# snphbaum/scikit-gpuppy

Measured on NVIDIA B200. Metric: fit_s_per_iter, lower is better.
Workload: dtype f64

## Files before the change

scikit-gpuppy_b200/csrc/factor.cuh:

```cuda
#pragma once
#include "dgemm_dmma.cuh"
#include "oz_gemm.cuh"
#include "leaf_blocked.cuh"

namespace gpk {


struct FactorCtx {
  double* A;
  double* X;
  long ld;
  double* dL;
  int* info;
  cudaStream_t st;
  cudaStream_t side = nullptr;
  cudaEvent_t* ev = nullptr;
  int* ev_next = nullptr;
  oz::Workspace* oz = nullptr;
  oz::Workspace* ovl_ws = nullptr;
  cudaStream_t* ovl_st = nullptr;
  int ovl_depths = 0;
};

inline int leaf_launch(const FactorCtx& c, int r0) {
// ... 80 lines not shown
  GPK_TRY((gemm_store_auto<LAY_KC, LAY_KC>(
      gemm_args(A21, ld, X11, ld, X21, ld, h2, h1, h1, 1.0, 0.0, K_UPTO_BJ, 0), c.st)));
  cudaStream_t tst = c.st;
  cudaEvent_t joined = nullptr;
  if (c.side) {
    cudaEvent_t forked = c.ev[(*c.ev_next)++];
    joined = c.ev[(*c.ev_next)++];
    GPK_CUDA_OK(cudaEventRecord(forked, c.st));
    GPK_CUDA_OK(cudaStreamWaitEvent(c.side, forked, 0));
    tst = c.side;
  }
  GPK_TRY((gemm_store_auto<LAY_KC, LAY_MC>(
      gemm_args(X21, ld, X11, ld, A21, ld, h2, h1, h1, 1.0, 0.0, K_FROM_BJ, 0), tst)));
  if (c.side) GPK_CUDA_OK(cudaEventRecord(joined, c.side));
  GPK_TRY((gemm_store_auto<LAY_KC, LAY_KC>(
      gemm_args(X21, ld, X21, ld, A22, ld, h2, h2, h1, -1.0, 1.0, K_FULL, 1), c.st)));
  GPK_TRY(potrf_inv_node(c, r0 + h1, h2, depth + 1));
  if (c.side) GPK_CUDA_OK(cudaStreamWaitEvent(c.st, joined, 0));
  GPK_TRY((gemm_store_auto<LAY_KC, LAY_MC>(
      gemm_args(X22, ld, A21, ld, X21, ld, h2, h1, h2, -1.0, 0.0, K_UPTO_BI, 0), c.st)));
  return 0;
}

inline int lauum_launch(const double* X, double* out, long ld, int npad, cudaStream_t st, oz::Workspace* oz = nullptr) {
  if (oz && npad >= oz->min_dim)
    return oz::gemm_f64(*oz, X, ld, 1, 1, npad, X, ld, 1, 1, npad, npad, out, ld, 1.0, 0.0, K_FROM_BI, 1, st);
  return gemm_store_auto<LAY_MC, LAY_MC>(
      gemm_args(X, ld, X, ld, out, ld, npad, npad, npad, 1.0, 0.0, K_FROM_BI, 1), st);
}

__global__ void __launch_bounds__(256) trmv_lower_kernel(const double* __restrict__ X, long ld, int npad,
                                                         const double* __restrict__ t, double* __restrict__ y) {
  const int row = blockIdx.x * 8 + (threadIdx.x >> 5);
  const int lane = threadIdx.x & 31;
  if (row >= npad) return;
  const double* Xr = X + (long)row * ld;
  double s = 0.0;
  for (int k = lane; k <= row; k += 32) s = fma(Xr[k], t[k], s);
  s = warp_sum(s);
  if (lane == 0) y[row] = s;
}

constexpr int TRMVT_ROWS = 512;
__global__ void __launch_bounds__(128) trmv_lower_T_partial_kernel(const double* __restrict__ X, long ld, int npad,
                                                                   const double* __restrict__ y,
                                                                   double* __restrict__ part) {
  const int c = blockIdx.x * 128 + threadIdx.x;
  const int r_begin = blockIdx.y * TRMVT_ROWS;
  const int r_end = min(npad, r_begin + TRMVT_ROWS);
// ... 72 lines not shown
```

scikit-gpuppy_b200/csrc/gpk.cu:

```cuda
#include "../../include/gpk.h"
#include "../../include/gpk_test.h"

#include <climits>
#include <new>
#include <vector>

#include "dgemm_dmma.cuh"
#include "factor.cuh"
#include "se_kernels.cuh"
#include "exact_kernels.cuh"
#include "periodic_kernels.cuh"

namespace gpk {
thread_local char g_err[512] = {0};
thread_local long g_launch_count = 0;
thread_local bool g_prof_on = false;
static thread_local std::vector<ProfPair> g_prof;
void prof_push(cudaEvent_t a, cudaEvent_t b) { g_prof.push_back(ProfPair{a, b}); }

struct Handle {
  int n = 0, d = 0, npad = 0;
  double *X = nullptr, *W = nullptr;
  bool own_X = false, own_W = false;
  double *x = nullptr, *xT = nullptr, *t = nullptr, *y = nullptr, *alpha = nullptr, *dL = nullptr;
// ... 10 lines not shown
  double theta[3 * MAX_D + 2];
  bool factored = false, have_inverse = false;
  bool matrix_state = false;
  double logdet = 0.0, quad = 0.0, alpha2 = 0.0;
  cudaStream_t st = nullptr;
  cudaStream_t side = nullptr;
  std::vector<cudaEvent_t> events;
  int ev_next = 0;
  bool oz_want = false;
  bool oz_on = false;
  int oz_moduli_req = 0;
  size_t oz_out_cap = 0;
  oz::Workspace oz;
  oz::Workspace ozq;
  oz::Operand xs;
  bool x_sliced = false;
  cudaStream_t chain_st = nullptr;
  std::vector<cudaStream_t> ovl_st;
  std::vector<oz::Workspace> ovl_ws;
  cudaEvent_t ev_in = nullptr, ev_out = nullptr;
  bool ovl_on = false;
  double* raw_pinned = nullptr;
  bool grad_pending = false;
};

thread_local int g_overlap_T = 1;

static void release_overlap(Handle* h) {
  for (auto& w : h->ovl_ws) w.release();
  h->ovl_ws.clear();
  for (auto& s : h->ovl_st) if (s) { cudaStreamSynchronize(s); cudaStreamDestroy(s); }
  h->ovl_st.clear();
  if (h->chain_st) { cudaStreamSynchronize(h->chain_st); cudaStreamDestroy(h->chain_st); h->chain_st = nullptr; }
  if (h->ev_in) { cudaEventDestroy(h->ev_in); h->ev_in = nullptr; }
  if (h->ev_out) { cudaEventDestroy(h->ev_out); h->ev_out = nullptr; }
  h->ovl_on = false;
}

static int ensure_overlap(Handle* h) {
  if (h->ovl_on || !h->oz_on || !g_overlap_T) return 0;
  int depths = 0;
  size_t need = 0;
  for (long hh = h->npad / 2 / TILE * TILE; hh >= h->oz.min_dim; hh = hh / 2 / TILE * TILE) {
    need += (size_t)h->oz.S * (hh + TILE) * (3 * (hh + TILE) + round_up_l(hh + TILE, 256)) + 6 * hh * sizeof(double);
    ++depths;
  }
// ... 104 lines not shown
  trmv_lower_kernel<<<(npad + 7) / 8, 256, 0, h->st>>>(h->X, npad, npad, b_pad, y);
  GPK_LAUNCH_OK();
  const int nchunks = (npad + TRMVT_ROWS - 1) / TRMVT_ROWS;
  GPK_TRY(ensure(&h->part, &h->part_elems, (size_t)nchunks * npad));
  dim3 grid(npad / 128, nchunks);
  trmv_lower_T_partial_kernel<<<grid, 128, 0, h->st>>>(h->X, npad, npad, y, h->part);
  GPK_LAUNCH_OK();
  sum_chunks_kernel<<<(npad + 255) / 256, 256, 0, h->st>>>(h->part, nchunks, npad, npad, out, 1.0, 0.0);
  GPK_LAUNCH_OK();
  return 0;
}

template <int DP>
static int launch_trace(Handle* h, int d0, int trb, int tre, double* partial) {
  const int nt = h->npad / TILE;
  const size_t smem = (size_t)2 * h->d * (TILE + 2) * sizeof(double);
  GPK_CUDA_OK(cudaFuncSetAttribute(grad_trace_kernel<DP>, cudaFuncAttributeMaxDynamicSharedMemorySize, (int)smem));
  dim3 grid(nt, tre - trb);
  grad_trace_kernel<DP><<<grid, 256, smem, h->st>>>(h->W, h->npad, h->alpha, h->x, h->n, h->d, d0, h->hyp, trb, partial);
  GPK_LAUNCH_OK();
  return 0;
}

static int trace_sums(Handle* h, int trb, int tre, double* raw_host, double* async_dst = nullptr) {
  const int d = h->d;
  const int nt = h->npad / TILE;
  for (int k = 0; k <= (h->kind == KIND_PERIODIC ? 3 * d + 2 : d + 2); ++k) raw_host[k] = 0.0;
  if (tre <= trb) return 0;
  if (h->kind != KIND_PERIODIC) {
    const int r0 = trb * TILE, r1 = (tre * TILE < h->n) ? tre * TILE : h->n;
    diag_sum_kernel<<<1, 256, 0, h->st>>>(h->W, h->npad, h->alpha, r0, r1, h->scal + 4);
    GPK_LAUNCH_OK();
    GPK_CUDA_OK(cudaMemcpyAsync(async_dst ? async_dst : raw_host + d + 1, h->scal + 4, 2 * sizeof(double),
                                cudaMemcpyDeviceToHost, h->st));
  }
  if (h->kind == KIND_PERIODIC) {
    const int DPp = d <= 4 ? 4 : d <= 8 ? 8 : 16;
    const int nc = 3 * DPp + 2;
    const long nsl = (long)nt * (tre - trb);
    GPK_TRY(ensure(&h->part, &h->part_elems, (size_t)nsl * nc + nc));
    double* psums = h->part + (size_t)nsl * nc;
    dim3 pgrid(nt, tre - trb);
    if (DPp == 4) periodic_trace_kernel<4><<<pgrid, 256, 0, h->st>>>(h->W, h->npad, h->alpha, h->x, h->n, d, h->hyp, trb, h->part);
    else if (DPp == 8) periodic_trace_kernel<8><<<pgrid, 256, 0, h->st>>>(h->W, h->npad, h->alpha, h->x, h->n, d, h->hyp, trb, h->part);
    else periodic_trace_kernel<16><<<pgrid, 256, 0, h->st>>>(h->W, h->npad, h->alpha, h->x, h->n, d, h->hyp, trb, h->part);
    GPK_LAUNCH_OK();
    col_sum_kernel<<<nc, 256, 0, h->st>>>(h->part, nsl, nc, psums);
    GPK_LAUNCH_OK();
    double ph[50];
    GPK_CUDA_OK(cudaMemcpyAsync(ph, psums, nc * sizeof(double), cudaMemcpyDeviceToHost, h->st));
    GPK_CUDA_OK(cudaStreamSynchronize(h->st));
    raw_host[0] = ph[0];
    for (int k = 0; k < d; ++k) {
      raw_host[1 + k] = ph[1 + k];
      raw_host[1 + d + k] = ph[1 + DPp + k];
      raw_host[1 + 2 * d + k] = ph[1 + 2 * DPp + k];
    }
    raw_host[3 * d + 1] = ph[3 * DPp + 1];
    raw_host[3 * d + 2] = 0.0;
    return 0;
  }
  int DP = d <= 4 ? 4 : d <= 8 ? 8 : d <= 16 ? 16 : 32;
  const long nslots = (long)nt * (tre - trb);
  const int nchunks = (d + DP - 1) / DP;
  GPK_TRY(ensure(&h->part, &h->part_elems, (size_t)nslots * (DP + 1) + (size_t)nchunks * (DP + 1)));
  double* sums = h->part + (size_t)nslots * (DP + 1);
  double host[2 * 33];
  for (int d0 = 0, ch = 0; d0 < d; d0 += DP, ++ch) {
    switch (DP) {
      case 4: GPK_TRY(launch_trace<4>(h, d0, trb, tre, h->part)); break;
      case 8: GPK_TRY(launch_trace<8>(h, d0, trb, tre, h->part)); break;
      case 16: GPK_TRY(launch_trace<16>(h, d0, trb, tre, h->part)); break;
      default: GPK_TRY(launch_trace<32>(h, d0, trb, tre, h->part)); break;
    }
    col_sum_kernel<<<DP + 1, 256, 0, h->st>>>(h->part, nslots, DP + 1, sums + ch * (DP + 1));
    GPK_LAUNCH_OK();
    double* dst = async_dst ? async_dst + 4 + ch * (DP + 1) : host + ch * 33;
    GPK_CUDA_OK(cudaMemcpyAsync(dst, sums + ch * (DP + 1), (DP + 1) * sizeof(double), cudaMemcpyDeviceToHost, h->st));
  }
  if (async_dst) return 0;
  GPK_CUDA_OK(cudaStreamSynchronize(h->st));
  for (int d0 = 0, ch = 0; d0 < d; d0 += DP, ++ch) {
    if (d0 == 0) raw_host[0] = host[0];
    for (int k = 0; k < DP && d0 + k < d; ++k) raw_host[1 + d0 + k] = host[ch * 33 + 1 + k];
  }
  return 0;
}

static void trace_unpack(const Handle* h, const double* pinned, double* raw_host) {
  const int d = h->d;
  const int DP = d <= 4 ? 4 : d <= 8 ? 8 : d <= 16 ? 16 : 32;
  raw_host[d + 1] = pinned[0];
  raw_host[d + 2] = pinned[1];
  for (int d0 = 0, ch = 0; d0 < d; d0 += DP, ++ch) {
    const double* src = pinned + 4 + ch * (DP + 1);
    if (d0 == 0) raw_host[0] = src[0];
    for (int k = 0; k < DP && d0 + k < d; ++k) raw_host[1 + d0 + k] = src[1 + k];
  }
}

static int ensure_route(Handle* h);

static int do_lauum(Handle* h) {
  if (h->have_inverse) return 0;
  GPK_TRY(ensure_route(h));
  h->x_sliced = false;
  GPK_TRY(lauum_launch(h->X, h->W, h->npad, h->npad, h->st, h->oz_on ? &h->oz : nullptr));
  h->have_inverse = true;
  return 0;
}

static bool same_theta(const Handle* h, const double* theta) {
  if (!h->factored || h->matrix_state) return false;
  return memcmp(h->theta, theta, sizeof(double) * theta_len(h->kind, h->d)) == 0;
}

static long batch_rows_for(const Handle* h, long want) {
  long cap = (long)(4.0e9 / (8.0 * h->npad));
  cap = cap / TILE * TILE;
  if (cap > 16384) cap = 16384;
  if (cap < TILE) cap = TILE;
  if (h->batch_rows > 0 && h->batch_rows < cap) cap = round_up_l(h->batch_rows, TILE);
  long r = round_up_l(want, TILE);
  return r < cap ? r : cap;
}

static int ensure_query_ws(Handle* h, long rows) {
  const long nbi = h->npad / TILE;
  GPK_TRY(ensure(&h->G, &h->G_elems, (size_t)rows * h->npad));
  size_t need = (size_t)nbi * rows + (size_t)nbi * (rows / 2);
  if (h->colsq_elems < need) {
// ... 160 lines not shown
  }
  Handle* h = new (std::nothrow) Handle();
  if (!h) return -3;
  const int rc = create_fill(h, n, d, Xbuf, Wbuf);
  if (rc != 0) {
    cudaGetLastError();
    gpk_destroy(reinterpret_cast<gpk_handle>(h));
    return rc;
  }
  *out = reinterpret_cast<gpk_handle>(h);
  return 0;
}

int gpk_destroy(gpk_handle h) {
  H_OR_FAIL(h);
  cudaStreamSynchronize(hh->st);
  if (hh->own_X) cudaFree(hh->X);
  if (hh->own_W) cudaFree(hh->W);
  cudaFree(hh->x); cudaFree(hh->xT); cudaFree(hh->t); cudaFree(hh->y); cudaFree(hh->alpha); cudaFree(hh->dL);
  cudaFree(hh->scal); cudaFree(hh->info);
  for (auto& e : hh->events) if (e) cudaEventDestroy(e);
  if (hh->side) { cudaStreamSynchronize(hh->side); cudaStreamDestroy(hh->side); }
  if (hh->part) cudaFree(hh->part);
  if (hh->G) cudaFree(hh->G);
  if (hh->colsq) cudaFree(hh->colsq);
  if (hh->dots) cudaFree(hh->dots);
  hh->oz.release();
  hh->ozq.release();
  release_overlap(hh);
  if (hh->raw_pinned) cudaFreeHost(hh->raw_pinned);
  delete hh;
  return 0;
}

int gpk_set_stream(gpk_handle h, void* stream) {
  H_OR_FAIL(h);
  hh->st = reinterpret_cast<cudaStream_t>(stream);
  return 0;
}

int gpk_set_kernel(gpk_handle h, int kind) {
  H_OR_FAIL(h);
  if (kind != KIND_SE && kind != KIND_PERIODIC) { snprintf(g_err, sizeof(g_err), "unknown kernel kind %d", kind); return -2; }
  if (kind == KIND_PERIODIC && hh->d > PER_MAX_D) {
    snprintf(g_err, sizeof(g_err), "the periodic covariance supports d <= %d", PER_MAX_D);
    return -2;
// ... 100 lines not shown
    cudaDeviceSynchronize();
    return rc_rec;
  }
  if (ovl) {
    GPK_CUDA_OK(cudaEventRecord(hh->ev_out, hh->chain_st));
    GPK_CUDA_OK(cudaStreamWaitEvent(hh->st, hh->ev_out, 0));
  }
  GPK_TRY(solve_one(hh, hh->t, hh->y, hh->alpha));
  nll_scalars_kernel<<<1, 256, 0, hh->st>>>(hh->dL, hh->y, hh->alpha, n, hh->scal);
  GPK_LAUNCH_OK();
  int info = 0;
  double sc[3];
  GPK_CUDA_OK(cudaMemcpyAsync(&info, hh->info, sizeof(int), cudaMemcpyDeviceToHost, hh->st));
  GPK_CUDA_OK(cudaMemcpyAsync(sc, hh->scal, 3 * sizeof(double), cudaMemcpyDeviceToHost, hh->st));
  GPK_CUDA_OK(cudaStreamSynchronize(hh->st));
  if (info != INT_MAX) {
    snprintf(g_err, sizeof(g_err), "leading minor %d of K is not positive definite", info);
    return info > 0 ? info : 1;
  }
  hh->logdet = sc[0]; hh->quad = sc[1]; hh->alpha2 = sc[2];
  return 0;
}

int gpk_factorize(gpk_handle h, const double* theta, int want_inverse) {
  H_OR_FAIL(h);
  if (!same_theta(hh, theta)) {
    hh->factored = false;
    hh->have_inverse = false;
    hh->x_sliced = false;
    hh->grad_pending = false;
    GPK_TRY(set_hyper(hh->hyp, theta, hh->d, hh->kind));
    GPK_TRY(ensure_route(hh));
    const int n = hh->n, npad = hh->npad;
    GPK_TRY(launch_se_tiles(hh->x, n, hh->x, n, hh->d, hh->hyp, hh->W, npad, npad, npad,
                            hh->kind == KIND_PERIODIC ? 2 : 1, 1, 1, hh->st));
    const int rc = factorize_W(hh);
    if (rc != 0) return rc;
    memcpy(hh->theta, theta, sizeof(double) * theta_len(hh->kind, hh->d));
    hh->factored = true;
    hh->matrix_state = false;
  }
  if (want_inverse) GPK_TRY(do_lauum(hh));
  return 0;
}

__global__ void __launch_bounds__(256) load_matrix_kernel(const double* __restrict__ K, long ldk, int n,
                                                          double* __restrict__ W, long ld, int npad) {
  const int c = blockIdx.x * 256 + threadIdx.x;
  const int r = blockIdx.y;
  if (c >= npad || (c >> 7) > (r >> 7)) return;
  W[(long)r * ld + c] = (r < n && c < n) ? K[(long)r * ldk + c] : (r == c ? 1.0 : 0.0);
}

int gpk_factorize_matrix(gpk_handle h, const double* K_dev, int64_t ldk, int want_inverse) {
  H_OR_FAIL(h);
  if (!K_dev || ldk < hh->n) { snprintf(g_err, sizeof(g_err), "gpk_factorize_matrix: bad matrix argument"); return -2; }
  hh->factored = false;
  hh->have_inverse = false;
  hh->x_sliced = false;
  GPK_TRY(ensure_route(hh));
  dim3 grid((hh->npad + 255) / 256, hh->npad);
  load_matrix_kernel<<<grid, 256, 0, hh->st>>>(K_dev, ldk, hh->n, hh->W, hh->npad, hh->npad);
  GPK_LAUNCH_OK();
  const int rc = factorize_W(hh);
  if (rc != 0) return rc;
  hh->factored = true;
// ... 15 lines not shown
  if (!hh->factored) { snprintf(g_err, sizeof(g_err), "not factored"); return -2; }
  *out = hh->logdet;
  return 0;
}

int gpk_grad_trace_partial(gpk_handle h, int64_t trb, int64_t tre, double* out) {
  H_OR_FAIL(h);
  if (!hh->factored || !hh->have_inverse || hh->matrix_state) { snprintf(g_err, sizeof(g_err), "inverse not available"); return -2; }
  if (hh->kind != KIND_SE) { snprintf(g_err, sizeof(g_err), "sharded trace: Gaussian covariance only"); return -2; }
  const int nt = hh->npad / TILE;
  if (trb < 0) trb = 0;
  if (tre > nt) tre = nt;
  return trace_sums(hh, (int)trb, (int)tre, out);
}

int gpk_nll_grad(gpk_handle h, const double* theta, double* nll, double* grad, int want_grad) {
  H_OR_FAIL(h);
  const bool prefetch = want_grad == 2 && hh->kind == KIND_SE;
  const bool cached = same_theta(hh, theta);
  if (!cached && hh->grad_pending) {
    GPK_CUDA_OK(cudaStreamSynchronize(hh->st));
    hh->grad_pending = false;
  }
  int rc = gpk_factorize(h, theta, want_grad == 1);
  if (rc != 0) return rc;
  const double two_pi = 6.283185307179586476925286766559;
  if (nll) *nll = 0.5 * hh->n * log(two_pi) + 0.5 * hh->logdet + 0.5 * hh->quad;
  if (prefetch && !hh->grad_pending) {
    if (!hh->raw_pinned) GPK_CUDA_OK(cudaMallocHost((void**)&hh->raw_pinned, (3 * MAX_D + 8) * sizeof(double)));
    GPK_TRY(do_lauum(hh));
    double unused[3 * MAX_D + 3];
    GPK_TRY(trace_sums(hh, 0, hh->npad / TILE, unused, hh->raw_pinned));
    hh->grad_pending = true;
    return 0;
  }
  if (want_grad == 1 && grad) {
    double raw[3 * MAX_D + 3];
    if (hh->grad_pending) {
      GPK_CUDA_OK(cudaStreamSynchronize(hh->st));
      trace_unpack(hh, hh->raw_pinned, raw);
      hh->grad_pending = false;
    } else {
      GPK_TRY(trace_sums(hh, 0, hh->npad / TILE, raw));
    }
    const int d = hh->d;
    grad[0] = 0.5 * raw[0];
    if (hh->kind == KIND_PERIODIC) {
      grad[1] = 0.5 * hh->hyp.vt * raw[3 * d + 1];
      for (int k = 0; k < d; ++k) {
        grad[2 + k] = -0.25 * hh->hyp.w[k] * raw[1 + k];
        grad[2 + d + k] = 0.5 * hh->hyp.pf[k] * hh->hyp.w2[k] * raw[1 + d + k];
        grad[2 + 2 * d + k] = -0.25 * hh->hyp.w2[k] * raw[1 + 2 * d + k];
      }
      return 0;
    }
    grad[1] = 0.5 * hh->hyp.vt * (raw[hh->d + 1] - raw[hh->d + 2]);
    for (int k = 0; k < hh->d; ++k) grad[2 + k] = -0.25 * hh->hyp.w[k] * raw[1 + k];
  }
  return 0;
}

int gpk_solve(gpk_handle h, const double* b, int64_t nrhs, double* out) {
  H_OR_FAIL(h);
  if (!hh->factored) { snprintf(g_err, sizeof(g_err), "not factored"); return -2; }
  const int npad = hh->npad, n = hh->n;
  GPK_TRY(ensure_query_ws(hh, TILE));
// ... 457 lines not shown
```

scikit-gpuppy_b200/csrc/oz_crt_planes.cuh:

```cuda

struct PlaneArgs {
  uint8_t* res; long res_ld; long res_plane;
  int M, N, K;
  int row_tile0;
  int krange, lower_only;
  int widen, band_cols;
  int nmod;
  unsigned int* phase;
  int* spill;
  int m[CRT_MAX_MODULI]; uint32_t magic[CRT_MAX_MODULI]; uint32_t u[CRT_MAX_MODULI];
};

constexpr int RECON_GROUPS = (CRT_MAX_MODULI + 3) / 4;

struct ReconArgs {
  const uint8_t* res; long res_ld; long res_plane;
  double* C; long ldc;
  const double* scA; const double* scB;
  double alpha, beta;
  int M, N, K;
  int row0;
  int krange, lower_only;
  int nmod;
  double p_scaled;
  double* colsq; double* pairdot; long ldo;
  uint32_t wp[2 * RECON_GROUPS][6];
};

constexpr int SPILL_SLOTS = 256;
constexpr int Q_BN = 256;
constexpr int Q_STAGES = 7;
constexpr int Q_STAGE_BYTES = 2 * TILE_BYTES;
constexpr int Q_SMEM_BYTES = Q_STAGES * Q_STAGE_BYTES + 1024 + 256;

__host__ __device__ __forceinline__ void planes_krange(int krange, int K, int bi2, int bx2, int& kb0, int& kb1) {
  kb0 = 0;
  kb1 = K / BK;
  switch (krange) {
    case K_UPTO_BJ: kb1 = (kb1 < 2 * bx2 + 2) ? kb1 : 2 * bx2 + 2; break;
    case K_FROM_BJ: kb0 = (kb1 < 2 * bx2) ? kb1 : 2 * bx2; break;
    case K_UPTO_BI: kb1 = (kb1 < 2 * bi2 + 2) ? kb1 : 2 * bi2 + 2; break;
    case K_FROM_BI: kb0 = (kb1 < 2 * bi2) ? kb1 : 2 * bi2; break;
    default: break;
  }
}

__global__ void __launch_bounds__(THREADS, 1)
oz_crt_planes_kernel(const __grid_constant__ CUtensorMap tmA, const __grid_constant__ CUtensorMap tmB,
                     const __grid_constant__ PlaneArgs p) {
  extern __shared__ uint8_t oz_smem_raw[];
// ... 205 lines not shown
        o[1] = make_uint4(pk[4], pk[5], pk[6], pk[7]);
      }
    }
  }
#undef SEG_MOD
#undef SEG_BEG
#undef SEG_END
  tc_fence_before();
  cluster_sync_all();
  if (warp == 2) tmem_dealloc_pair(tmem_base, TMEM_COLS);
}

__device__ __forceinline__ uint32_t dp2a_lo(uint32_t a, uint32_t b, uint32_t c) {
  uint32_t d;
  asm("dp2a.lo.u32.u32 %0, %1, %2, %3;" : "=r"(d) : "r"(a), "r"(b), "r"(c));
  return d;
}
__device__ __forceinline__ uint32_t dp2a_hi(uint32_t a, uint32_t b, uint32_t c) {
  uint32_t d;
  asm("dp2a.hi.u32.u32 %0, %1, %2, %3;" : "=r"(d) : "r"(a), "r"(b), "r"(c));
  return d;
}

template <int EPI, int NG>
__global__ void __launch_bounds__(256, 4) oz_crt_reconstruct_kernel(const __grid_constant__ ReconArgs p) {
  const int lane = threadIdx.x & 31, warp = threadIdx.x >> 5;
  const int bjc = blockIdx.x;
  const long lrow = (long)blockIdx.y * 8 + warp;
  const long grow = (long)p.row0 + lrow;
  const long gcol = (long)bjc * 128 + lane * 4;
  const int bi = (int)(grow >> 7), bi2 = (int)(grow >> 8), bx2 = bjc >> 1;
  if (EPI == OZ_EPI_STORE && p.lower_only && bjc > bi) return;
  int kb0, kb1;
  planes_krange(p.krange, p.K, bi2, bx2, kb0, kb1);
  const bool computed = (kb1 > kb0) && !(p.lower_only && 2 * bx2 > 2 * bi2 + 1);

  uint32_t acc[4][6];
#pragma unroll
  for (int x = 0; x < 4; ++x)
#pragma unroll
    for (int j = 0; j < 6; ++j) acc[x][j] = 0u;
  if (computed) {
    const uint8_t* src = p.res + lrow * p.res_ld + gcol;
    uint32_t q[NG * 4];
#pragma unroll
    for (int i = 0; i < NG * 4; ++i) {
      q[i] = (i < 4 * (NG - 1) || i < p.nmod) ? __ldcs(reinterpret_cast<const uint32_t*>(src)) : 0u;
      src += p.res_plane;
    }
#pragma unroll
    for (int g = 0; g < NG; ++g) {
      {
        const uint32_t ab_lo = __byte_perm(q[4 * g], q[4 * g + 1], 0x5140), ab_hi = __byte_perm(q[4 * g], q[4 * g + 1], 0x7362);
        const uint32_t cd_lo = __byte_perm(q[4 * g + 2], q[4 * g + 3], 0x5140),
                       cd_hi = __byte_perm(q[4 * g + 2], q[4 * g + 3], 0x7362);
        const uint32_t t[4] = {__byte_perm(ab_lo, cd_lo, 0x5410), __byte_perm(ab_lo, cd_lo, 0x7632),
                               __byte_perm(ab_hi, cd_hi, 0x5410), __byte_perm(ab_hi, cd_hi, 0x7632)};
#pragma unroll
        for (int e = 0; e < 4; ++e)
#pragma unroll
          for (int j = 0; j < 6; ++j) {
            uint32_t v = acc[e][j];
            v = dp2a_lo(p.wp[2 * g][j], t[e], v);
            v = dp2a_hi(p.wp[2 * g + 1][j], t[e], v);
            acc[e][j] = v;
          }
      }
    }
  }
  const bool row_ok = grow < p.M;
  const bool col_ok = gcol < p.N;
  const double sa = row_ok ? p.scA[grow] * p.p_scaled : 0.0;
  double v[4];
#pragma unroll
  for (int x = 0; x < 4; ++x) {
    const unsigned long long t0 = ((unsigned long long)acc[x][1] << 16) + acc[x][0];
    const unsigned long long t1 = ((unsigned long long)acc[x][3] << 16) + acc[x][2] + (t0 >> 32);
    const unsigned long long t2 = ((unsigned long long)acc[x][5] << 16) + acc[x][4] + (t1 >> 32);
    const long long hi = (long long)((t2 << 32) | (t1 & 0xffffffffull));
    const double frac = fma((double)hi, 4294967296.0, (double)(uint32_t)t0);
    v[x] = col_ok ? sa * p.scB[gcol + x] * frac : 0.0;
  }
  if (EPI == OZ_EPI_STORE) {
    if (row_ok && col_ok) {
      double* crow = p.C + grow * p.ldc + gcol;
#pragma unroll
      for (int x = 0; x < 4; x += 2) {
        double2 o;
        o.x = p.alpha * v[x];
        o.y = p.alpha * v[x + 1];
        if (p.beta != 0.0) {
          const double2 old = *reinterpret_cast<const double2*>(crow + x);
          o.x = fma(p.beta, old.x, o.x);
          o.y = fma(p.beta, old.y, o.y);
        }
        *reinterpret_cast<double2*>(crow + x) = o;
      }
    }
  } else {
    __shared__ double vrow[8][128];
#pragma unroll
    for (int x = 0; x < 4; ++x) vrow[warp][lane * 4 + x] = v[x];
    __syncthreads();
    double sq = 0.0, pd = 0.0;
#pragma unroll
    for (int x = 0; x < 4; ++x) {
      sq = fma(v[x], v[x], sq);
      pd = fma(v[x], vrow[warp ^ 1][lane * 4 + x], pd);
    }
#pragma unroll
    for (int off = 1; off < 32; off <<= 1) {
      sq += __shfl_xor_sync(0xffffffffu, sq, off);
      pd += __shfl_xor_sync(0xffffffffu, pd, off);
    }
    if (lane == 0 && row_ok) {
      p.colsq[(long)bjc * p.ldo + grow] = sq;
      if (!(grow & 1)) p.pairdot[(long)bjc * (p.ldo / 2) + (grow >> 1)] = pd;
    }
  }
}
```

scikit-gpuppy_b200/csrc/oz_gemm.cuh:

```cuda
#pragma once
#include <cuda.h>

#include "dgemm_dmma.cuh"
#include "oz_crt_tables.h"

namespace gpk {
namespace oz {

constexpr int BM = 128, BN = 128, BK = 128;
constexpr int TILE_BYTES = BM * BK;
constexpr int EPI_WARPS = 8;
constexpr int THREADS = 64 + EPI_WARPS * 32;
constexpr int TMEM_COLS = 512;

constexpr int OZ_EPI_STORE = 0;
constexpr int OZ_EPI_ROWSQ = 1;

__device__ __forceinline__ uint32_t smem_u32(const void* p) { return (uint32_t)__cvta_generic_to_shared(p); }

__device__ __forceinline__ void mbar_init(uint64_t* bar, uint32_t count) {
  asm volatile("mbarrier.init.shared::cta.b64 [%0], %1;" ::"r"(smem_u32(bar)), "r"(count) : "memory");
}
__device__ __forceinline__ void fence_barrier_init() {
  asm volatile("fence.mbarrier_init.release.cluster;" ::: "memory");
}
__device__ __forceinline__ void mbar_expect_tx(uint64_t* bar, uint32_t bytes) {
  asm volatile("mbarrier.arrive.expect_tx.shared::cta.b64 _, [%0], %1;" ::"r"(smem_u32(bar)), "r"(bytes) : "memory");
}
__device__ __forceinline__ void mbar_arrive(uint64_t* bar) {
  asm volatile("mbarrier.arrive.shared::cta.b64 _, [%0];" ::"r"(smem_u32(bar)) : "memory");
}
__device__ __forceinline__ bool mbar_try_wait(uint64_t* bar, uint32_t parity) {
  uint32_t ok;
  asm volatile(
      "{\n\t.reg .pred p;\n\t"
      "mbarrier.try_wait.parity.shared::cta.b64 p, [%1], %2;\n\t"
      "selp.u32 %0, 1, 0, p;\n\t}\n"
      : "=r"(ok)
      : "r"(smem_u32(bar)), "r"(parity)
// ... 317 lines not shown
  if (!trans) {
    oz_absmax_rows_kernel<<<op.rows, 256, 0, st>>>(src, ld, op.K, lower, mx);
    GPK_LAUNCH_OK();
    const long chunks = (long)op.rows * (op.K >> 4);
    oz_residue_rows_kernel<<<(unsigned)((chunks + 255) / 256), 256, 0, st>>>(src, ld, op.rows, op.K, lower, op.S,
                                                                            op.bits, zero_fill_extra(op.K), mx, op.sl, op.sc);
    GPK_LAUNCH_OK();
  } else {
    GPK_CUDA_OK(cudaMemsetAsync(mx, 0, (size_t)op.rows * sizeof(unsigned long long), st));
    dim3 g1(op.rows / 32, (op.K + 1023) / 1024);
    oz_absmax_cols_kernel<<<g1, 256, 0, st>>>(src, ld, op.K, lower, mx);
    GPK_LAUNCH_OK();
    dim3 g2(op.rows / 32, (op.K + 127) / 128);
    oz_residue_cols_kernel<<<g2, 256, 0, st>>>(src, ld, op.rows, op.K, lower, op.S, op.bits, zero_fill_extra(op.K), mx, op.sl, op.sc);
    GPK_LAUNCH_OK();
  }
  return 0;
}

thread_local int g_position_lock = 2;

inline int gemm_sliced(const Operand& A, const Operand& B, double* C, long ldc, double alpha, double beta, int krange,
                       int lower_only, cudaStream_t st, int epi = OZ_EPI_STORE, double* colsq = nullptr,
                       double* pairdot = nullptr, long ldo = 0) {
  if (A.K != B.K || A.S != B.S) {
    snprintf(g_err, sizeof(g_err), "gemm_sliced: operand mismatch K %d/%d moduli %d/%d", A.K, B.K, A.S, B.S);
    return -2;
  }
  if (A.bits != B.bits || A.bits != crt_bits(A.K, A.S)) {
    snprintf(g_err, sizeof(g_err), "gemm_sliced: operand widths %d/%d do not match K=%d", A.bits, B.bits, A.K);
    return -2;
  }
  const long Nc = ((long)B.rows + Q_BN - 1) / Q_BN * Q_BN;
  const size_t per_row = (size_t)A.S * (size_t)Nc;
  const long panel = (long)(A.out_cap / per_row) / 256 * 256;
  if (!A.out || panel < 256) {
    snprintf(g_err, sizeof(g_err), "gemm_sliced: the residue-plane buffer (%zu bytes) cannot hold a 256-row panel of %ld columns",
             A.out_cap, Nc);
    return -4;
  }
  static bool configured_on[GPK_MAX_DEVICES] = {};
  bool& configured = configured_on[current_device_slot()];
  if (!configured) {
    GPK_CUDA_OK(cudaFuncSetAttribute(oz_crt_planes_kernel, cudaFuncAttributeMaxDynamicSharedMemorySize, Q_SMEM_BYTES));
    configured = true;
  }
  CUtensorMap tmA, tmB;
  GPK_TRY(make_tmap(&tmA, A.sl, A.rows, A.K, A.S, BM));
  GPK_TRY(make_tmap(&tmB, B.sl, B.rows, B.K, B.S, BM));
  const CrtSet& cs = crt_set(A.S);
  PlaneArgs g;
  memset(&g, 0, sizeof(g));
  g.res = A.out; g.res_ld = Nc;
// ... 38 lines not shown
    r.row0 = (int)row0;
    r.res_plane = g.res_plane;
    long ncol_tiles = Nc / Q_BN;
    if (lower_only && (row0 + rows_pad) / Q_BN < ncol_tiles) ncol_tiles = (row0 + rows_pad) / Q_BN;
    g.phase = phase_dev + (phase_next++ & 63);
    GPK_CUDA_OK(cudaMemsetAsync(g.phase, 0, sizeof(unsigned int), st));
    cudaLaunchConfig_t cfg;
    memset(&cfg, 0, sizeof(cfg));
    cudaLaunchAttribute attr[1];
    attr[0].id = cudaLaunchAttributeClusterDimension;
    attr[0].val.clusterDim.x = 2;
    attr[0].val.clusterDim.y = 1;
    attr[0].val.clusterDim.z = 1;
    cfg.gridDim = dim3((unsigned)(2 * ncol_tiles), (unsigned)(rows_pad / 256));
    cfg.blockDim = dim3(THREADS);
    cfg.dynamicSmemBytes = Q_SMEM_BYTES;
    cfg.stream = st;
    cfg.attrs = attr;
    cfg.numAttrs = 1;
    GPK_CUDA_OK(cudaLaunchKernelEx(&cfg, oz_crt_planes_kernel, tmA, tmB, g));
    GPK_LAUNCH_OK();
    long ncol_blocks = B.rows / 128;
    if (lower_only && (row0 + rows) / 128 < ncol_blocks) ncol_blocks = (row0 + rows) / 128;
    dim3 rg((unsigned)ncol_blocks, (unsigned)(rows / 8));
    const int ng = (A.S + 3) / 4;
    const bool store = epi == OZ_EPI_STORE;
    auto kernel = (ng <= 2) ? (store ? oz_crt_reconstruct_kernel<OZ_EPI_STORE, 2> : oz_crt_reconstruct_kernel<OZ_EPI_ROWSQ, 2>)
                : (ng == 3) ? (store ? oz_crt_reconstruct_kernel<OZ_EPI_STORE, 3> : oz_crt_reconstruct_kernel<OZ_EPI_ROWSQ, 3>)
                : (ng == 4) ? (store ? oz_crt_reconstruct_kernel<OZ_EPI_STORE, 4> : oz_crt_reconstruct_kernel<OZ_EPI_ROWSQ, 4>)
                            : (store ? oz_crt_reconstruct_kernel<OZ_EPI_STORE, 5> : oz_crt_reconstruct_kernel<OZ_EPI_ROWSQ, 5>);
    kernel<<<rg, 256, 0, st>>>(r);
    GPK_LAUNCH_OK();
  }
  if (g_prof_on) {
    GPK_CUDA_OK(cudaEventRecord(e1, st));
    prof_push(e0, e1);
  }
  return 0;
}

struct Workspace {
  int8_t* buf = nullptr; size_t cap = 0, top = 0;
  double* sc = nullptr; size_t sc_cap = 0, sc_top = 0;
  unsigned long long* mx = nullptr; size_t mx_cap = 0;
  uint8_t* out = nullptr; size_t out_cap = 0;
  int S = CRT_MIN_MODULI;
  int min_dim = 2048;
  void reset() { top = 0; sc_top = 0; }
// ... 26 lines not shown
      sc = nullptr; sc_cap = 0;
      if (cudaMalloc((void**)&sc, rows_total * sizeof(double)) != cudaSuccess) { cudaGetLastError(); return -1; }
      sc_cap = rows_total;
    }
    if (rows_max > mx_cap) {
      if (mx) cudaFree(mx);
      mx = nullptr; mx_cap = 0;
      if (cudaMalloc((void**)&mx, rows_max * sizeof(unsigned long long)) != cudaSuccess) { cudaGetLastError(); return -1; }
      mx_cap = rows_max;
    }
    return 0;
  }
  void release() {
    if (buf) cudaFree(buf);
    if (sc) cudaFree(sc);
    if (mx) cudaFree(mx);
    if (out) cudaFree(out);
    buf = nullptr; sc = nullptr; mx = nullptr; out = nullptr; cap = sc_cap = mx_cap = out_cap = 0;
  }
};

inline int gemm_f64(Workspace& ws, const double* A, long lda, int transA, int lowerA, int M, const double* B, long ldb,
                    int transB, int lowerB, int N, int K, double* C, long ldc, double alpha, double beta, int krange,
                    int lower_only, cudaStream_t st) {
  ws.reset();
  Operand a = ws.alloc(M, K);
  const bool same = (A == B && lda == ldb && transA == transB && lowerA == lowerB && M == N);
  Operand b = same ? a : ws.alloc(N, K);
  if (!a.sl || !b.sl) {
    snprintf(g_err, sizeof(g_err), "gemm_f64: residue workspace too small for %d x %d and %d x %d operands", M, K, N, K);
    return -4;
  }
  GPK_TRY(slice_operand(A, lda, transA, lowerA, a, ws.mx, st));
  if (same) b = a;
  else GPK_TRY(slice_operand(B, ldb, transB, lowerB, b, ws.mx, st));
  return gemm_sliced(a, b, C, ldc, alpha, beta, krange, lower_only, st);
}

}
}
```

Before: 0.3087.

## Fuse gradient trace reduction into INT8 CRT reconstruction epilogue of LAUUM

Adds a reconstruct kernel for the Ozaki INT8 LAUUM that, while writing K^-1 tiles, also accumulates the squared-exponential gradient trace sums per tile into a partial buffer. trace_sums then skips the separate grad_trace_kernel pass and only column-sums the fused partials. The aim is to avoid re-reading the full K^-1 matrix from memory for the gradient. In exchange the reconstruct kernel does more per-thread work with higher register and shared-memory use, and the partial buffer needs a memset on every call.

```diff
diff --git a/scikit-gpuppy_b200/csrc/factor.cuh b/scikit-gpuppy_b200/csrc/factor.cuh
--- a/scikit-gpuppy_b200/csrc/factor.cuh
+++ b/scikit-gpuppy_b200/csrc/factor.cuh
@@ -126,9 +126,14 @@
   return 0;
 }
 
-inline int lauum_launch(const double* X, double* out, long ld, int npad, cudaStream_t st, oz::Workspace* oz = nullptr) {
+inline int lauum_launch(const double* X, double* out, long ld, int npad, cudaStream_t st, oz::Workspace* oz = nullptr,
+                        const oz::TraceArgs* trace = nullptr) {
   if (oz && npad >= oz->min_dim)
-    return oz::gemm_f64(*oz, X, ld, 1, 1, npad, X, ld, 1, 1, npad, npad, out, ld, 1.0, 0.0, K_FROM_BI, 1, st);
+    return oz::gemm_f64(*oz, X, ld, 1, 1, npad, X, ld, 1, 1, npad, npad, out, ld, 1.0, 0.0, K_FROM_BI, 1, st, trace);
+  if (trace) {
+    snprintf(g_err, sizeof(g_err), "lauum_launch: the trace epilogue needs the INT8 route");
+    return -2;
+  }
   return gemm_store_auto<LAY_MC, LAY_MC>(
       gemm_args(X, ld, X, ld, out, ld, npad, npad, npad, 1.0, 0.0, K_FROM_BI, 1), st);
 }
diff --git a/scikit-gpuppy_b200/csrc/gpk.cu b/scikit-gpuppy_b200/csrc/gpk.cu
--- a/scikit-gpuppy_b200/csrc/gpk.cu
+++ b/scikit-gpuppy_b200/csrc/gpk.cu
@@ -56,6 +56,8 @@
   bool ovl_on = false;
   double* raw_pinned = nullptr;
   bool grad_pending = false;
+  double* tpart = nullptr; size_t tpart_elems = 0;
+  bool inverse_traced = false;
 };
 
 thread_local int g_overlap_T = 1;
@@ -206,11 +208,15 @@
   return 0;
 }
 
-static int trace_sums(Handle* h, int trb, int tre, double* raw_host, double* async_dst = nullptr) {
+static int trace_sums(Handle* h, int trb, int tre, double* raw_host, double* async_dst = nullptr, bool fused = false) {
   const int d = h->d;
   const int nt = h->npad / TILE;
   for (int k = 0; k <= (h->kind == KIND_PERIODIC ? 3 * d + 2 : d + 2); ++k) raw_host[k] = 0.0;
   if (tre <= trb) return 0;
+  if (fused && (!h->inverse_traced || trb != 0 || tre != nt || h->kind != KIND_SE || d > oz::TRACE_MAX_D)) {
+    snprintf(g_err, sizeof(g_err), "trace_sums: no gradient sums were formed with this K^-1");
+    return -2;
+  }
   if (h->kind != KIND_PERIODIC) {
     const int r0 = trb * TILE, r1 = (tre * TILE < h->n) ? tre * TILE : h->n;
     diag_sum_kernel<<<1, 256, 0, h->st>>>(h->W, h->npad, h->alpha, r0, r1, h->scal + 4);
@@ -251,13 +257,15 @@
   double* sums = h->part + (size_t)nslots * (DP + 1);
   double host[2 * 33];
   for (int d0 = 0, ch = 0; d0 < d; d0 += DP, ++ch) {
-    switch (DP) {
-      case 4: GPK_TRY(launch_trace<4>(h, d0, trb, tre, h->part)); break;
-      case 8: GPK_TRY(launch_trace<8>(h, d0, trb, tre, h->part)); break;
-      case 16: GPK_TRY(launch_trace<16>(h, d0, trb, tre, h->part)); break;
-      default: GPK_TRY(launch_trace<32>(h, d0, trb, tre, h->part)); break;
-    }
-    col_sum_kernel<<<DP + 1, 256, 0, h->st>>>(h->part, nslots, DP + 1, sums + ch * (DP + 1));
+    if (!fused) {
+      switch (DP) {
+        case 4: GPK_TRY(launch_trace<4>(h, d0, trb, tre, h->part)); break;
+        case 8: GPK_TRY(launch_trace<8>(h, d0, trb, tre, h->part)); break;
+        case 16: GPK_TRY(launch_trace<16>(h, d0, trb, tre, h->part)); break;
+        default: GPK_TRY(launch_trace<32>(h, d0, trb, tre, h->part)); break;
+      }
+    }
+    col_sum_kernel<<<DP + 1, 256, 0, h->st>>>(fused ? h->tpart : h->part, nslots, DP + 1, sums + ch * (DP + 1));
     GPK_LAUNCH_OK();
     double* dst = async_dst ? async_dst + 4 + ch * (DP + 1) : host + ch * 33;
     GPK_CUDA_OK(cudaMemcpyAsync(dst, sums + ch * (DP + 1), (DP + 1) * sizeof(double), cudaMemcpyDeviceToHost, h->st));
@@ -285,12 +293,28 @@
 
 static int ensure_route(Handle* h);
 
-static int do_lauum(Handle* h) {
+static int do_lauum(Handle* h, bool trace = false) {
   if (h->have_inverse) return 0;
   GPK_TRY(ensure_route(h));
   h->x_sliced = false;
-  GPK_TRY(lauum_launch(h->X, h->W, h->npad, h->npad, h->st, h->oz_on ? &h->oz : nullptr));
+  const bool int8 = h->oz_on && h->npad >= h->oz.min_dim;
+  oz::TraceArgs ta;
+  const bool fuse = trace && int8 && h->kind == KIND_SE && h->d <= oz::TRACE_MAX_D;
+  if (fuse) {
+    const long nt = h->npad / TILE;
+    const int DP = oz::trace_dp(h->d);
+    GPK_TRY(ensure(&h->tpart, &h->tpart_elems, (size_t)(nt * nt) * (DP + 1)));
+    GPK_CUDA_OK(cudaMemsetAsync(h->tpart, 0, (size_t)(nt * nt) * (DP + 1) * sizeof(double), h->st));
+    memset(&ta, 0, sizeof(ta));
+    ta.alpha = h->alpha; ta.x = h->x; ta.n = h->n; ta.d = h->d;
+    ta.v = h->hyp.v;
+    for (int k = 0; k < h->d; ++k) ta.w[k] = h->hyp.w[k];
+    ta.part = h->tpart;
+  }
+  h->inverse_traced = false;
+  GPK_TRY(lauum_launch(h->X, h->W, h->npad, h->npad, h->st, int8 ? &h->oz : nullptr, fuse ? &ta : nullptr));
   h->have_inverse = true;
+  h->inverse_traced = fuse;
   return 0;
 }
 
@@ -497,6 +521,7 @@
   for (auto& e : hh->events) if (e) cudaEventDestroy(e);
   if (hh->side) { cudaStreamSynchronize(hh->side); cudaStreamDestroy(hh->side); }
   if (hh->part) cudaFree(hh->part);
+  if (hh->tpart) cudaFree(hh->tpart);
   if (hh->G) cudaFree(hh->G);
   if (hh->colsq) cudaFree(hh->colsq);
   if (hh->dots) cudaFree(hh->dots);
@@ -643,8 +668,7 @@
   return 0;
 }
 
-int gpk_factorize(gpk_handle h, const double* theta, int want_inverse) {
-  H_OR_FAIL(h);
+static int factorize(Handle* hh, const double* theta, int want_inverse, bool trace) {
   if (!same_theta(hh, theta)) {
     hh->factored = false;
     hh->have_inverse = false;
@@ -661,8 +685,13 @@
     hh->factored = true;
     hh->matrix_state = false;
   }
-  if (want_inverse) GPK_TRY(do_lauum(hh));
-  return 0;
+  if (want_inverse) GPK_TRY(do_lauum(hh, trace));
+  return 0;
+}
+
+int gpk_factorize(gpk_handle h, const double* theta, int want_inverse) {
+  H_OR_FAIL(h);
+  return factorize(hh, theta, want_inverse, false);
 }
 
 __global__ void __launch_bounds__(256) load_matrix_kernel(const double* __restrict__ K, long ldk, int n,
@@ -724,15 +753,15 @@
     GPK_CUDA_OK(cudaStreamSynchronize(hh->st));
     hh->grad_pending = false;
   }
-  int rc = gpk_factorize(h, theta, want_grad == 1);
+  int rc = factorize(hh, theta, want_grad == 1, want_grad == 1 && grad);
   if (rc != 0) return rc;
   const double two_pi = 6.283185307179586476925286766559;
   if (nll) *nll = 0.5 * hh->n * log(two_pi) + 0.5 * hh->logdet + 0.5 * hh->quad;
   if (prefetch && !hh->grad_pending) {
     if (!hh->raw_pinned) GPK_CUDA_OK(cudaMallocHost((void**)&hh->raw_pinned, (3 * MAX_D + 8) * sizeof(double)));
-    GPK_TRY(do_lauum(hh));
+    GPK_TRY(do_lauum(hh, true));
     double unused[3 * MAX_D + 3];
-    GPK_TRY(trace_sums(hh, 0, hh->npad / TILE, unused, hh->raw_pinned));
+    GPK_TRY(trace_sums(hh, 0, hh->npad / TILE, unused, hh->raw_pinned, hh->inverse_traced));
     hh->grad_pending = true;
     return 0;
   }
@@ -743,7 +772,7 @@
       trace_unpack(hh, hh->raw_pinned, raw);
       hh->grad_pending = false;
     } else {
-      GPK_TRY(trace_sums(hh, 0, hh->npad / TILE, raw));
+      GPK_TRY(trace_sums(hh, 0, hh->npad / TILE, raw, nullptr, hh->inverse_traced));
     }
     const int d = hh->d;
     grad[0] = 0.5 * raw[0];
diff --git a/scikit-gpuppy_b200/csrc/oz_crt_planes.cuh b/scikit-gpuppy_b200/csrc/oz_crt_planes.cuh
--- a/scikit-gpuppy_b200/csrc/oz_crt_planes.cuh
+++ b/scikit-gpuppy_b200/csrc/oz_crt_planes.cuh
@@ -26,6 +26,14 @@
   double* colsq; double* pairdot; long ldo;
   uint32_t wp[2 * RECON_GROUPS][6];
 };
+
+constexpr int TRACE_MAX_D = 32;
+struct TraceArgs {
+  const double* alpha; const double* x; int n, d;
+  double v; double w[TRACE_MAX_D];
+  double* part;
+};
+inline int trace_dp(int d) { return d <= 4 ? 4 : d <= 8 ? 8 : d <= 16 ? 16 : 32; }
 
 constexpr int SPILL_SLOTS = 256;
 constexpr int Q_BN = 256;
@@ -277,6 +285,56 @@
   return d;
 }
 
+template <int NG>
+__device__ __forceinline__ void crt_values(const ReconArgs& p, long lrow, long grow, long gcol, bool computed,
+                                           double (&v)[4]) {
+  uint32_t acc[4][6];
+#pragma unroll
+  for (int x = 0; x < 4; ++x)
+#pragma unroll
+    for (int j = 0; j < 6; ++j) acc[x][j] = 0u;
+  if (computed) {
+    const uint8_t* src = p.res + lrow * p.res_ld + gcol;
+    uint32_t q[NG * 4];
+#pragma unroll
+    for (int i = 0; i < NG * 4; ++i) {
+      q[i] = (i < 4 * (NG - 1) || i < p.nmod) ? __ldcs(reinterpret_cast<const uint32_t*>(src)) : 0u;
+      src += p.res_plane;
+    }
+#pragma unroll
+    for (int g = 0; g < NG; ++g) {
+      {
+        const uint32_t ab_lo = __byte_perm(q[4 * g], q[4 * g + 1], 0x5140), ab_hi = __byte_perm(q[4 * g], q[4 * g + 1], 0x7362);
+        const uint32_t cd_lo = __byte_perm(q[4 * g + 2], q[4 * g + 3], 0x5140),
+                       cd_hi = __byte_perm(q[4 * g + 2], q[4 * g + 3], 0x7362);
+        const uint32_t t[4] = {__byte_perm(ab_lo, cd_lo, 0x5410), __byte_perm(ab_lo, cd_lo, 0x7632),
+                               __byte_perm(ab_hi, cd_hi, 0x5410), __byte_perm(ab_hi, cd_hi, 0x7632)};
+#pragma unroll
+        for (int e = 0; e < 4; ++e)
+#pragma unroll
+          for (int j = 0; j < 6; ++j) {
+            uint32_t v = acc[e][j];
+            v = dp2a_lo(p.wp[2 * g][j], t[e], v);
+            v = dp2a_hi(p.wp[2 * g + 1][j], t[e], v);
+            acc[e][j] = v;
+          }
+      }
+    }
+  }
+  const bool row_ok = grow < p.M;
+  const bool col_ok = gcol < p.N;
+  const double sa = row_ok ? p.scA[grow] * p.p_scaled : 0.0;
+#pragma unroll
+  for (int x = 0; x < 4; ++x) {
+    const unsigned long long t0 = ((unsigned long long)acc[x][1] << 16) + acc[x][0];
+    const unsigned long long t1 = ((unsigned long long)acc[x][3] << 16) + acc[x][2] + (t0 >> 32);
+    const unsigned long long t2 = ((unsigned long long)acc[x][5] << 16) + acc[x][4] + (t1 >> 32);
+    const long long hi = (long long)((t2 << 32) | (t1 & 0xffffffffull));
+    const double frac = fma((double)hi, 4294967296.0, (double)(uint32_t)t0);
+    v[x] = col_ok ? sa * p.scB[gcol + x] * frac : 0.0;
+  }
+}
+
 template <int EPI, int NG>
 __global__ void __launch_bounds__(256, 4) oz_crt_reconstruct_kernel(const __grid_constant__ ReconArgs p) {
   const int lane = threadIdx.x & 31, warp = threadIdx.x >> 5;
@@ -289,53 +347,10 @@
   int kb0, kb1;
   planes_krange(p.krange, p.K, bi2, bx2, kb0, kb1);
   const bool computed = (kb1 > kb0) && !(p.lower_only && 2 * bx2 > 2 * bi2 + 1);
-
-  uint32_t acc[4][6];
-#pragma unroll
-  for (int x = 0; x < 4; ++x)
-#pragma unroll
-    for (int j = 0; j < 6; ++j) acc[x][j] = 0u;
-  if (computed) {
-    const uint8_t* src = p.res + lrow * p.res_ld + gcol;
-    uint32_t q[NG * 4];
-#pragma unroll
-    for (int i = 0; i < NG * 4; ++i) {
-      q[i] = (i < 4 * (NG - 1) || i < p.nmod) ? __ldcs(reinterpret_cast<const uint32_t*>(src)) : 0u;
-      src += p.res_plane;
-    }
-#pragma unroll
-    for (int g = 0; g < NG; ++g) {
-      {
-        const uint32_t ab_lo = __byte_perm(q[4 * g], q[4 * g + 1], 0x5140), ab_hi = __byte_perm(q[4 * g], q[4 * g + 1], 0x7362);
-        const uint32_t cd_lo = __byte_perm(q[4 * g + 2], q[4 * g + 3], 0x5140),
-                       cd_hi = __byte_perm(q[4 * g + 2], q[4 * g + 3], 0x7362);
-        const uint32_t t[4] = {__byte_perm(ab_lo, cd_lo, 0x5410), __byte_perm(ab_lo, cd_lo, 0x7632),
-                               __byte_perm(ab_hi, cd_hi, 0x5410), __byte_perm(ab_hi, cd_hi, 0x7632)};
-#pragma unroll
-        for (int e = 0; e < 4; ++e)
-#pragma unroll
-          for (int j = 0; j < 6; ++j) {
-            uint32_t v = acc[e][j];
-            v = dp2a_lo(p.wp[2 * g][j], t[e], v);
-            v = dp2a_hi(p.wp[2 * g + 1][j], t[e], v);
-            acc[e][j] = v;
-          }
-      }
-    }
-  }
+  double v[4];
+  crt_values<NG>(p, lrow, grow, gcol, computed, v);
   const bool row_ok = grow < p.M;
   const bool col_ok = gcol < p.N;
-  const double sa = row_ok ? p.scA[grow] * p.p_scaled : 0.0;
-  double v[4];
-#pragma unroll
-  for (int x = 0; x < 4; ++x) {
-    const unsigned long long t0 = ((unsigned long long)acc[x][1] << 16) + acc[x][0];
-    const unsigned long long t1 = ((unsigned long long)acc[x][3] << 16) + acc[x][2] + (t0 >> 32);
-    const unsigned long long t2 = ((unsigned long long)acc[x][5] << 16) + acc[x][4] + (t1 >> 32);
-    const long long hi = (long long)((t2 << 32) | (t1 & 0xffffffffull));
-    const double frac = fma((double)hi, 4294967296.0, (double)(uint32_t)t0);
-    v[x] = col_ok ? sa * p.scB[gcol + x] * frac : 0.0;
-  }
   if (EPI == OZ_EPI_STORE) {
     if (row_ok && col_ok) {
       double* crow = p.C + grow * p.ldc + gcol;
@@ -374,3 +389,121 @@
     }
   }
 }
+
+constexpr int TRACE_XLD = TILE + 2;
+template <int NG, int DP>
+__global__ void __launch_bounds__(256, (DP <= 16) ? 2 : 1)
+oz_crt_reconstruct_trace_kernel(const __grid_constant__ ReconArgs p, const __grid_constant__ TraceArgs t) {
+  const int bj = blockIdx.x, bi = p.row0 / TILE + (int)blockIdx.y;
+  if (bj > bi) return;
+  extern __shared__ __align__(16) double tsm[];
+  __shared__ __align__(16) double kv[2][8][TILE];
+  __shared__ double al_a[TILE];
+  __shared__ double red[8];
+  const int tid = threadIdx.x, lane = tid & 31, warp = tid >> 5;
+  const int d = t.d, n = t.n;
+  const int row0 = bi * TILE, col0 = bj * TILE;
+  double* xa = tsm;
+  double* xb = tsm + (long)d * TRACE_XLD;
+  for (int idx = tid; idx < TILE * d; idx += 256) {
+    const int r = idx / d, k = idx % d;
+    xa[k * TRACE_XLD + r] = (row0 + r < n) ? t.x[(long)(row0 + r) * d + k] : 0.0;
+    xb[k * TRACE_XLD + r] = (col0 + r < n) ? t.x[(long)(col0 + r) * d + k] : 0.0;
+  }
+  if (tid < TILE) al_a[tid] = (row0 + tid < n) ? t.alpha[row0 + tid] : 0.0;
+
+  const long gcol = (long)col0 + lane * 4;
+  int kb0, kb1;
+  planes_krange(p.krange, p.K, bi >> 1, bj >> 1, kb0, kb1);
+  const bool computed = (kb1 > kb0) && !(p.lower_only && 2 * (bj >> 1) > 2 * (bi >> 1) + 1);
+  const long lrow0 = (long)row0 - p.row0 + (warp & 3) + 64 * (warp >> 2);
+  const int c = tid & (TILE - 1), hw = (tid >> 7) * 4, rh = (tid >> 7) * 64;
+  const bool col_ok = (col0 + c) < n;
+  const bool diag_tile = (bi == bj);
+  const double alc = col_ok ? t.alpha[col0 + c] : 0.0;
+  double g0 = 0.0;
+  double gk[DP];
+#pragma unroll
+  for (int k = 0; k < DP; ++k) gk[k] = 0.0;
+  __syncthreads();
+
+  for (int g = 0; g < TILE / 8; ++g) {
+    const long lrow = lrow0 + 4 * g, grow = (long)p.row0 + lrow;
+    double v[4];
+    crt_values<NG>(p, lrow, grow, gcol, computed, v);
+    double o[4];
+#pragma unroll
+    for (int x = 0; x < 4; ++x) o[x] = p.alpha * v[x];
+    if (grow < p.M && gcol < p.N) {
+      double* crow = p.C + grow * p.ldc + gcol;
+      *reinterpret_cast<double2*>(crow) = make_double2(o[0], o[1]);
+      *reinterpret_cast<double2*>(crow + 2) = make_double2(o[2], o[3]);
+    }
+    *reinterpret_cast<double2*>(&kv[g & 1][warp][lane * 4]) = make_double2(o[0], o[1]);
+    *reinterpret_cast<double2*>(&kv[g & 1][warp][lane * 4 + 2]) = make_double2(o[2], o[3]);
+    if (computed && g + 1 < TILE / 8 && lane < p.nmod)
+      asm volatile("prefetch.global.L2 [%0];" ::"l"(p.res + (lrow + 4) * p.res_ld + (long)col0 + (long)lane * p.res_plane));
+    __syncthreads();
+
+#pragma unroll
+    for (int s = 0; s < 2; ++s) {
+      const int r0 = rh + 4 * g + 2 * s;
+      double m[2], dist[2], sq[2][DP];
+#pragma unroll
+      for (int i = 0; i < 2; ++i) {
+        const int r = r0 + i;
+        const double kcur = kv[g & 1][hw + 2 * s + i][c];
+        const bool ok = col_ok && (row0 + r) < n && !(diag_tile && c > r);
+        const double sym = (diag_tile && c == r) ? 1.0 : 2.0;
+        m[i] = ok ? sym * (kcur - al_a[r] * alc) : 0.0;
+        dist[i] = 0.0;
+      }
+#pragma unroll
+      for (int k = 0; k < DP; ++k) {
+        if (k < d) {
+          const double bv = xb[k * TRACE_XLD + c];
+          const double wk = t.w[k];
+          const double2 av = *reinterpret_cast<const double2*>(&xa[k * TRACE_XLD + r0]);
+          const double d0v = av.x - bv, d1v = av.y - bv;
+          sq[0][k] = d0v * d0v;
+          sq[1][k] = d1v * d1v;
+          dist[0] = fma(wk, sq[0][k], dist[0]);
+          dist[1] = fma(wk, sq[1][k], dist[1]);
+        } else {
+          sq[0][k] = 0.0;
+          sq[1][k] = 0.0;
+        }
+      }
+#pragma unroll
+      for (int i = 0; i < 2; ++i) {
+        const double pk = m[i] * t.v * exp(-0.5 * dist[i]);
+        g0 += pk;
+#pragma unroll
+        for (int k = 0; k < DP; ++k) gk[k] = fma(pk, sq[i][k], gk[k]);
+      }
+    }
+  }
+
+  double* out = t.part + ((long)bi * (p.N / TILE) + bj) * (DP + 1);
+  double sum = block_sum_256(g0, red);
+  if (tid == 0) out[0] = sum;
+#pragma unroll
+  for (int k = 0; k < DP; ++k) {
+    sum = block_sum_256(gk[k], red);
+    if (tid == 0) out[1 + k] = sum;
+  }
+}
+
+template <int NG>
+inline int launch_recon_trace(dim3 grid, const ReconArgs& r, const TraceArgs& t, cudaStream_t st) {
+  const size_t smem = (size_t)2 * t.d * TRACE_XLD * sizeof(double);
+  const int dp = trace_dp(t.d);
+  auto kernel = dp == 4 ? oz_crt_reconstruct_trace_kernel<NG, 4>
+              : dp == 8 ? oz_crt_reconstruct_trace_kernel<NG, 8>
+              : dp == 16 ? oz_crt_reconstruct_trace_kernel<NG, 16>
+                         : oz_crt_reconstruct_trace_kernel<NG, 32>;
+  GPK_CUDA_OK(cudaFuncSetAttribute(kernel, cudaFuncAttributeMaxDynamicSharedMemorySize, (int)smem));
+  kernel<<<grid, 256, smem, st>>>(r, t);
+  GPK_LAUNCH_OK();
+  return 0;
+}
diff --git a/scikit-gpuppy_b200/csrc/oz_gemm.cuh b/scikit-gpuppy_b200/csrc/oz_gemm.cuh
--- a/scikit-gpuppy_b200/csrc/oz_gemm.cuh
+++ b/scikit-gpuppy_b200/csrc/oz_gemm.cuh
@@ -15,6 +15,7 @@
 
 constexpr int OZ_EPI_STORE = 0;
 constexpr int OZ_EPI_ROWSQ = 1;
+constexpr int OZ_EPI_TRACE = 2;
 
 __device__ __forceinline__ uint32_t smem_u32(const void* p) { return (uint32_t)__cvta_generic_to_shared(p); }
 
@@ -378,13 +379,19 @@
 
 inline int gemm_sliced(const Operand& A, const Operand& B, double* C, long ldc, double alpha, double beta, int krange,
                        int lower_only, cudaStream_t st, int epi = OZ_EPI_STORE, double* colsq = nullptr,
-                       double* pairdot = nullptr, long ldo = 0) {
+                       double* pairdot = nullptr, long ldo = 0, const TraceArgs* trace = nullptr) {
   if (A.K != B.K || A.S != B.S) {
     snprintf(g_err, sizeof(g_err), "gemm_sliced: operand mismatch K %d/%d moduli %d/%d", A.K, B.K, A.S, B.S);
     return -2;
   }
   if (A.bits != B.bits || A.bits != crt_bits(A.K, A.S)) {
     snprintf(g_err, sizeof(g_err), "gemm_sliced: operand widths %d/%d do not match K=%d", A.bits, B.bits, A.K);
+    return -2;
+  }
+  if (epi == OZ_EPI_TRACE && (!trace || trace->d < 1 || trace->d > TRACE_MAX_D || alpha != 1.0 || beta != 0.0 ||
+                              !lower_only || A.rows != B.rows)) {
+    snprintf(g_err, sizeof(g_err), "gemm_sliced: the trace epilogue takes a square lower product with alpha 1, beta 0, d <= %d",
+             TRACE_MAX_D);
     return -2;
   }
   const long Nc = ((long)B.rows + Q_BN - 1) / Q_BN * Q_BN;
@@ -469,8 +476,16 @@
     GPK_LAUNCH_OK();
     long ncol_blocks = B.rows / 128;
     if (lower_only && (row0 + rows) / 128 < ncol_blocks) ncol_blocks = (row0 + rows) / 128;
+    const int ng = (A.S + 3) / 4;
+    if (epi == OZ_EPI_TRACE) {
+      const dim3 tg((unsigned)ncol_blocks, (unsigned)(rows / TILE));
+      GPK_TRY((ng <= 2) ? launch_recon_trace<2>(tg, r, *trace, st)
+              : (ng == 3) ? launch_recon_trace<3>(tg, r, *trace, st)
+              : (ng == 4) ? launch_recon_trace<4>(tg, r, *trace, st)
+                          : launch_recon_trace<5>(tg, r, *trace, st));
+      continue;
+    }
     dim3 rg((unsigned)ncol_blocks, (unsigned)(rows / 8));
-    const int ng = (A.S + 3) / 4;
     const bool store = epi == OZ_EPI_STORE;
     auto kernel = (ng <= 2) ? (store ? oz_crt_reconstruct_kernel<OZ_EPI_STORE, 2> : oz_crt_reconstruct_kernel<OZ_EPI_ROWSQ, 2>)
                 : (ng == 3) ? (store ? oz_crt_reconstruct_kernel<OZ_EPI_STORE, 3> : oz_crt_reconstruct_kernel<OZ_EPI_ROWSQ, 3>)
@@ -543,7 +558,7 @@
 
 inline int gemm_f64(Workspace& ws, const double* A, long lda, int transA, int lowerA, int M, const double* B, long ldb,
                     int transB, int lowerB, int N, int K, double* C, long ldc, double alpha, double beta, int krange,
-                    int lower_only, cudaStream_t st) {
+                    int lower_only, cudaStream_t st, const TraceArgs* trace = nullptr) {
   ws.reset();
   Operand a = ws.alloc(M, K);
   const bool same = (A == B && lda == ldb && transA == transB && lowerA == lowerB && M == N);
@@ -555,8 +570,9 @@
   GPK_TRY(slice_operand(A, lda, transA, lowerA, a, ws.mx, st));
   if (same) b = a;
   else GPK_TRY(slice_operand(B, ldb, transB, lowerB, b, ws.mx, st));
-  return gemm_sliced(a, b, C, ldc, alpha, beta, krange, lower_only, st);
-}
-
-}
-}
+  return gemm_sliced(a, b, C, ldc, alpha, beta, krange, lower_only, st, trace ? OZ_EPI_TRACE : OZ_EPI_STORE, nullptr,
+                     nullptr, 0, trace);
+}
+
+}
+}
```

Result: no change. 0.3062 (median of 6 runs) (-0.8%).
